# aredden/torch-bnb-fp4

Measured on AMD Instinct MI355X. Metric: FP4 dequant GB/s (% HBM peak) + fused-GEMV us/layer, 4096x4096 bf16, higher is better.
Workload: dtype bf16

## Files before the change

### torch-bnb-fp4_amd/csrc/gemv_common.h

```cpp
#pragma once

#include "fp4_common.h"

namespace fp4 {
namespace {

constexpr uint32_t kF16HiLo = 0x4A482C00u, kF16HiHi = 0x42404644u;
constexpr uint32_t kE4M3Lo = 0x54501800u, kE4M3Hi = 0x44404C48u;

__device__ __forceinline__ uint32_t perm(uint32_t hi, uint32_t lo, uint32_t sel) { return __builtin_amdgcn_perm(hi, lo, sel); }

template <int DT>
__device__ __forceinline__ void decode8(uint32_t q, uint32_t (&P)[4]) {
#if defined(FP4_EXP_BITOP3) || defined(FP4_EXP_RELAID)
    if constexpr (DT == FP4_DTYPE_BF16) {
        uint32_t m80;
        asm("v_mov_b32 %0, 0x80808080" : "=v"(m80));
        const uint32_t mhi = __builtin_amdgcn_bitop3_b32(q, m80, perm(kE4M3Hi, kE4M3Lo, (q >> 4) & 0x07070707u), 0xEA);
        const uint32_t mlo = __builtin_amdgcn_bitop3_b32(q << 4, m80, perm(kE4M3Hi, kE4M3Lo, q & 0x07070707u), 0xEA);
        P[0] = __builtin_bit_cast(uint32_t, __builtin_amdgcn_cvt_scalef32_pk_bf16_fp8(mhi, 1.0f, false));
        P[1] = __builtin_bit_cast(uint32_t, __builtin_amdgcn_cvt_scalef32_pk_bf16_fp8(mhi, 1.0f, true));
        P[2] = __builtin_bit_cast(uint32_t, __builtin_amdgcn_cvt_scalef32_pk_bf16_fp8(mlo, 1.0f, false));
        P[3] = __builtin_bit_cast(uint32_t, __builtin_amdgcn_cvt_scalef32_pk_bf16_fp8(mlo, 1.0f, true));
        return;
    }
#endif
    const uint32_t lo_sel = q & 0x07070707u;
    const uint32_t hi_sel = (q >> 4) & 0x07070707u;
    const uint32_t lo_sgn = (q & 0x08080808u) << 4;
    const uint32_t hi_sgn = q & 0x80808080u;
    if constexpr (DT == FP4_DTYPE_F16) {
        const uint32_t mhi = perm(kF16HiHi, kF16HiLo, hi_sel) | hi_sgn;
        const uint32_t mlo = perm(kF16HiHi, kF16HiLo, lo_sel) | lo_sgn;
        P[0] = perm(0u, mhi, 0x010C000Cu);
        P[1] = perm(0u, mhi, 0x030C020Cu);
        P[2] = perm(0u, mlo, 0x010C000Cu);
        P[3] = perm(0u, mlo, 0x030C020Cu);
    } else {
        const uint32_t mhi = perm(kE4M3Hi, kE4M3Lo, hi_sel) | hi_sgn;
        const uint32_t mlo = perm(kE4M3Hi, kE4M3Lo, lo_sel) | lo_sgn;
        P[0] = __builtin_bit_cast(uint32_t, __builtin_amdgcn_cvt_scalef32_pk_bf16_fp8(mhi, 1.0f, false));
        P[1] = __builtin_bit_cast(uint32_t, __builtin_amdgcn_cvt_scalef32_pk_bf16_fp8(mhi, 1.0f, true));
        P[2] = __builtin_bit_cast(uint32_t, __builtin_amdgcn_cvt_scalef32_pk_bf16_fp8(mlo, 1.0f, false));
        P[3] = __builtin_bit_cast(uint32_t, __builtin_amdgcn_cvt_scalef32_pk_bf16_fp8(mlo, 1.0f, true));
    }
}

template <int DT>
__device__ __forceinline__ float dot2(uint32_t a, uint32_t b, float c) {
    if constexpr (DT == FP4_DTYPE_F16)
        return __builtin_amdgcn_fdot2(__builtin_bit_cast(f16x2, a), __builtin_bit_cast(f16x2, b), c, false);
    else
        return __builtin_amdgcn_fdot2_f32_bf16(__builtin_bit_cast(bf16x2, a), __builtin_bit_cast(bf16x2, b), c, false);
}

template <int CTRL>
__device__ __forceinline__ float dpp_add(float v) {
    const int moved = __builtin_amdgcn_update_dpp(0, __builtin_bit_cast(int, v), CTRL, 0xF, 0xF, false);
    return v + __builtin_bit_cast(float, moved);
}
__device__ __forceinline__ float wave_sum(float v) {
    v = dpp_add<0x128>(v);
    v = dpp_add<0x124>(v);
    v = dpp_add<0x122>(v);
    v = dpp_add<0x121>(v);
    v += __builtin_bit_cast(float, __builtin_amdgcn_ds_swizzle(__builtin_bit_cast(int, v), 0x401F));
    const float a = __builtin_bit_cast(float, __builtin_amdgcn_readlane(__builtin_bit_cast(int, v), 0));
    const float b = __builtin_bit_cast(float, __builtin_amdgcn_readlane(__builtin_bit_cast(int, v), 32));
    return a + b;
}

constexpr int kModeOutF32 = 1;
constexpr int kModeSiluMulPairs = 2;

template <int DT>
__device__ __forceinline__ void store_row(uint16_t *out, const uint16_t *bias, const uint16_t *residual, int row, float sum,
                                          int mode = 0) {
    if (mode & kModeOutF32) {
        reinterpret_cast<float *>(out)[row] = sum;
        return;
    }
    uint16_t t = from_f32<DT>(sum);
    if (bias) t = from_f32<DT>(to_f32<DT>(t) + to_f32<DT>(bias[row]));
    if (residual) t = from_f32<DT>(to_f32<DT>(t) + to_f32<DT>(residual[row]));
    out[row] = t;
}

template <int DT>
__device__ __forceinline__ void store_silu_mul(uint16_t *out, const uint16_t *bias, const uint16_t *residual, int pair,
                                               float gate_sum, float up_sum) {
    uint16_t g = from_f32<DT>(gate_sum), u = from_f32<DT>(up_sum);
    if (bias) {
        g = from_f32<DT>(to_f32<DT>(g) + to_f32<DT>(bias[2 * pair]));
        u = from_f32<DT>(to_f32<DT>(u) + to_f32<DT>(bias[2 * pair + 1]));
    }
    const float gf = to_f32<DT>(g);
    const uint16_t s = from_f32<DT>(gf / (1.0f + expf(-gf)));
    uint16_t t = from_f32<DT>(to_f32<DT>(s) * to_f32<DT>(u));
    if (residual) t = from_f32<DT>(to_f32<DT>(t) + to_f32<DT>(residual[pair]));
    out[pair] = t;
}

template <int DT>
__device__ __forceinline__ void store_small(uint16_t *out, const uint16_t *bias, const uint16_t *residual, int64_t b, int row, int M,
                                            float sum) {
    if (bias) sum += to_f32<DT>(bias[row]);
    uint16_t t = from_f32<DT>(sum);
    if (residual) t = from_f32<DT>(to_f32<DT>(t) + to_f32<DT>(residual[b * M + row]));
    out[b * M + row] = t;
}

template <int DT>
__device__ __forceinline__ void store_small_silu_mul(uint16_t *out, const uint16_t *bias, const uint16_t *residual, int64_t b, int pair,
                                                     int M_half, float gate_sum, float up_sum) {
    if (bias) gate_sum += to_f32<DT>(bias[2 * pair]), up_sum += to_f32<DT>(bias[2 * pair + 1]);
    const float gf = to_f32<DT>(from_f32<DT>(gate_sum));
    const uint16_t s = from_f32<DT>(gf / (1.0f + expf(-gf)));
    uint16_t t = from_f32<DT>(to_f32<DT>(s) * to_f32<DT>(from_f32<DT>(up_sum)));
    if (residual) t = from_f32<DT>(to_f32<DT>(t) + to_f32<DT>(residual[b * M_half + pair]));
    out[b * M_half + pair] = t;
}

}
}
```

### torch-bnb-fp4_amd/csrc/gemv_fp4.hip

```cpp
#include <atomic>

#include "gemv_common.h"

#ifdef FP4_EXP_STAMPS
__device__ unsigned long long *fp4_exp_stamps = nullptr;
extern "C" int fp4_exp_set_stamps(void *buf) {
    return (int)hipMemcpyToSymbol(HIP_SYMBOL(fp4_exp_stamps), &buf, sizeof(buf));
}
#define FP4_STAMP(i)                                                                                        \
    do {                                                                                                    \
        __builtin_amdgcn_sched_barrier(0);                                                                  \
        const unsigned long long t_ = __builtin_amdgcn_s_memrealtime();                                     \
        if ((threadIdx.x & 63) == 0 && fp4_exp_stamps)                                                      \
            fp4_exp_stamps[(size_t(blockIdx.x) * WAVES + (threadIdx.x >> 6)) * 4 + (i)] = t_;               \
        __builtin_amdgcn_sched_barrier(0);                                                                  \
    } while (0)
#else
#define FP4_STAMP(i)
#endif

namespace fp4 {

namespace {

template <int ROWS, int UNROLL>
struct WTrip {
    u32x4 wq[UNROLL][ROWS];
    float am[UNROLL][ROWS];
};

template <int ROWS, int UNROLL>
__device__ __forceinline__ void issue_trip(WTrip<ROWS, UNROLL> &t, const u32x4 *__restrict__ Wv,
                                           const float *__restrict__ absmax, const int (&rows)[ROWS], int c0, int C,
                                           int bs_shift) {
#pragma unroll
    for (int u = 0; u < UNROLL; ++u) {
        const int c = c0 + 64 * u;
        const int cc = c < C ? c : C - 1;
#pragma unroll
        for (int r = 0; r < ROWS; ++r) {
            const int64_t chunk = int64_t(rows[r]) * C + cc;
            t.wq[u][r] = __builtin_nontemporal_load(Wv + chunk);
            const float a = absmax[(chunk << 5) >> bs_shift];
            t.am[u][r] = c < C ? a : 0.0f;
        }
    }
}

template <int DT, int ROWS, int UNROLL>
__device__ __forceinline__ void consume_trip(const WTrip<ROWS, UNROLL> &t, const u32x4 *s_x4, int c0, int C,
                                             float (&acc)[ROWS]) {
#pragma unroll
    for (int u = 0; u < UNROLL; ++u) {
        const int c = c0 + 64 * u;
        const int cc = c < C ? c : C - 1;
        u32x4 xd[4];
#pragma unroll
        for (int g = 0; g < 4; ++g) xd[g] = s_x4[g * C + cc];
#pragma unroll
        for (int r = 0; r < ROWS; ++r) {
            float s[4] = {0.0f, 0.0f, 0.0f, 0.0f};
#pragma unroll
            for (int g = 0; g < 4; ++g) {
                uint32_t P[4];
                decode8<DT>(t.wq[u][r][g], P);
                s[g] = dot2<DT>(P[0], xd[g].x, s[g]);
                s[g] = dot2<DT>(P[1], xd[g].y, s[g]);
                s[g] = dot2<DT>(P[2], xd[g].z, s[g]);
                s[g] = dot2<DT>(P[3], xd[g].w, s[g]);
            }
            acc[r] = __builtin_fmaf((s[0] + s[1]) + (s[2] + s[3]), t.am[u][r], acc[r]);
        }
    }
}

template <int DT, int ROWS, int WAVES, int UNROLL>
__global__ __launch_bounds__(WAVES * 64) void gemv16_kernel(const uint16_t *__restrict__ x,
                                                            const uint8_t *__restrict__ W,
                                                            const float *__restrict__ absmax,
                                                            const uint16_t *__restrict__ bias,
                                                            const uint16_t *residual, uint16_t *out, int M, int K,
                                                            int bs_shift, int mode) {
    extern __shared__ __attribute__((aligned(16))) uint32_t s_x[];
    u32x4 *s_x4 = reinterpret_cast<u32x4 *>(s_x);
    const int tid = threadIdx.x;
    const int lane = tid & 63;
    const int wave = tid >> 6;
    const int C = K >> 5;
    constexpr int kStride = 64 * UNROLL;
    const int trips = (C + kStride - 1) / kStride;

    const int row0 = (blockIdx.x * WAVES + wave) * ROWS;
    int rows[ROWS];
#pragma unroll
    for (int r = 0; r < ROWS; ++r) rows[r] = (row0 + r < M) ? row0 + r : M - 1;
    const u32x4 *Wv = reinterpret_cast<const u32x4 *>(W);

    constexpr int kXPre = 2;
    u32x4 xpre[kXPre];
#pragma unroll
    for (int i = 0; i < kXPre; ++i) {
        const int p = tid + i * WAVES * 64;
        xpre[i] = reinterpret_cast<const u32x4 *>(x)[p < 4 * C ? p : 4 * C - 1];
    }
    WTrip<ROWS, UNROLL> ta, tb;
    issue_trip<ROWS, UNROLL>(ta, Wv, absmax, rows, lane, C, bs_shift);

    auto stage = [&](int p, const u32x4 w) {
        u32x4 d;
        d.x = perm(w.y, w.x, 0x05040100u);
        d.y = perm(w.w, w.z, 0x05040100u);
        d.z = perm(w.y, w.x, 0x07060302u);
        d.w = perm(w.w, w.z, 0x07060302u);
        s_x4[(p & 3) * C + (p >> 2)] = d;
    };
#pragma unroll
    for (int i = 0; i < kXPre; ++i) {
        const int p = tid + i * WAVES * 64;
        if (p < 4 * C) stage(p, xpre[i]);
    }
    for (int p = tid + kXPre * WAVES * 64; p < 4 * C; p += WAVES * 64) stage(p, reinterpret_cast<const u32x4 *>(x)[p]);
    __syncthreads();

    float acc[ROWS];
#pragma unroll
    for (int r = 0; r < ROWS; ++r) acc[r] = 0.0f;

    for (int t = 0;;) {
        if (t + 1 < trips) issue_trip<ROWS, UNROLL>(tb, Wv, absmax, rows, lane + (t + 1) * kStride, C, bs_shift);
        consume_trip<DT, ROWS, UNROLL>(ta, s_x4, lane + t * kStride, C, acc);
        if (++t >= trips) break;
        if (t + 1 < trips) issue_trip<ROWS, UNROLL>(ta, Wv, absmax, rows, lane + (t + 1) * kStride, C, bs_shift);
        consume_trip<DT, ROWS, UNROLL>(tb, s_x4, lane + t * kStride, C, acc);
        if (++t >= trips) break;
    }

#pragma unroll
    for (int r = 0; r < ROWS; ++r) {
        const float total = wave_sum(acc[r]) * (1.0f / 12.0f);
        if (lane == 0 && row0 + r < M) store_row<DT>(out, bias, residual, row0 + r, total, mode);
    }
}

template <int DT, int KSPLIT, int G, int ITERS, int WAVES = 4>
__global__ __launch_bounds__(WAVES * 64, (G >= 4 ? 4 : 1)) void gemv16_regx_kernel(const uint16_t *__restrict__ x, const uint8_t *__restrict__ W,
                                                          const float *__restrict__ absmax,
                                                          const uint16_t *__restrict__ bias, const uint16_t *residual,
                                                          uint16_t *out, int M, int K, int bs_shift, int mode) {
    constexpr int RG = WAVES / KSPLIT;
    constexpr int kRowsPerBlock = 2 * RG * ITERS;
    __shared__ float s_part[kRowsPerBlock][KSPLIT];
    FP4_STAMP(0);
    const int tid = threadIdx.x;
    const int lane = tid & 63;
    const int wave = tid >> 6;
    const int kw = wave % KSPLIT, rw = wave / KSPLIT;
    const int half = lane >> 5, l32 = lane & 31;
    const int C = K >> 5;
    const int row_base = blockIdx.x * kRowsPerBlock;

    int cidx[G];
    bool live[G];
#pragma unroll
    for (int g = 0; g < G; ++g) {
        const int c = g * (32 * KSPLIT) + kw * 32 + l32;
        live[g] = c < C;
        cidx[g] = live[g] ? c : C - 1;
    }
    constexpr bool GMAJOR = G > 1;
    u32x4 xraw[G][4];
    u32x4 wq[ITERS][G];
    float am[ITERS][G];
    int rowi[ITERS], rclamp[ITERS];
#pragma unroll
    for (int it = 0; it < ITERS; ++it) {
        const int local = 2 * (it * RG + rw) + half;
        const int row = row_base + local;
        rowi[it] = local;
        rclamp[it] = row < M ? row : M - 1;
    }
    auto load_x = [&](int g) {
#pragma unroll
        for (int q = 0; q < 4; ++q) {
#ifdef FP4_ABL_NOX
            xraw[g][q] = u32x4{uint32_t(cidx[g]), 0x3c003c00u, uint32_t(q), 0x3c003c00u};
#else
            xraw[g][q] = reinterpret_cast<const u32x4 *>(x)[cidx[g] * 4 + q];
#endif
        }
    };
    const __amdgpu_buffer_rsrc_t rsrc_w = __builtin_amdgcn_make_buffer_rsrc(const_cast<uint8_t *>(W), 0, int((uint32_t(M) * uint32_t(C)) << 4), 0x00020000);
    const __amdgpu_buffer_rsrc_t rsrc_a =
        __builtin_amdgcn_make_buffer_rsrc(const_cast<float *>(absmax), 0, int(((uint32_t(M) * uint32_t(C)) >> (bs_shift - 5)) << 2), 0x00020000);
    auto load_w = [&](int it, int g) {
        const uint32_t chunk = uint32_t(rclamp[it]) * uint32_t(C) + uint32_t(cidx[g]);
        wq[it][g] = __builtin_bit_cast(u32x4, __builtin_amdgcn_raw_buffer_load_b128(rsrc_w, int(chunk << 4), 0, 2));
#ifdef FP4_ABL_NOABSMAX
        const float a = 0.5f;
#else
        const float a = __builtin_bit_cast(float, __builtin_amdgcn_raw_buffer_load_b32(rsrc_a, int((chunk >> (bs_shift - 5)) << 2), 0, 0));
#endif
        am[it][g] = live[g] ? a : 0.0f;
    };
    if constexpr (GMAJOR) {
#pragma unroll
        for (int g = 0; g < G; ++g) {
            load_x(g);
#pragma unroll
            for (int it = 0; it < ITERS; ++it) load_w(it, g);
        }
    } else {
#pragma unroll
        for (int g = 0; g < G; ++g) load_x(g);
#pragma unroll
        for (int it = 0; it < ITERS; ++it) {
#pragma unroll
            for (int g = 0; g < G; ++g) load_w(it, g);
        }
    }
    FP4_STAMP(1);
    u32x4 xd[G][4];
    auto permute_x = [&](int g) {
#pragma unroll
        for (int q = 0; q < 4; ++q) {
            const u32x4 w = xraw[g][q];
#ifdef FP4_EXP_RELAID
            xd[g][q] = u32x4{w.x, w.z, w.y, w.w};
#else
            xd[g][q].x = perm(w.y, w.x, 0x05040100u);
            xd[g][q].y = perm(w.w, w.z, 0x05040100u);
            xd[g][q].z = perm(w.y, w.x, 0x07060302u);
            xd[g][q].w = perm(w.w, w.z, 0x07060302u);
#endif
        }
    };
    if constexpr (!GMAJOR) {
#pragma unroll
        for (int g = 0; g < G; ++g) permute_x(g);
    }
    float pacc[ITERS];
#pragma unroll
    for (int it = 0; it < ITERS; ++it) pacc[it] = 0.0f;
    auto consume = [&](int it, int g) {
        float s[2] = {0.0f, 0.0f};
#ifdef FP4_ABL_NOCOMPUTE
#pragma unroll
        for (int q = 0; q < 4; ++q) s[q & 1] = __builtin_bit_cast(float, (wq[it][g][q] ^ xd[g][q].x) & 0x3fffffffu);
#else
#pragma unroll
        for (int q = 0; q < 4; ++q) {
            uint32_t P[4];
            decode8<DT>(wq[it][g][q], P);
            s[q & 1] = dot2<DT>(P[0], xd[g][q].x, s[q & 1]);
            s[q & 1] = dot2<DT>(P[1], xd[g][q].y, s[q & 1]);
            s[q & 1] = dot2<DT>(P[2], xd[g][q].z, s[q & 1]);
            s[q & 1] = dot2<DT>(P[3], xd[g][q].w, s[q & 1]);
        }
#endif
        pacc[it] = __builtin_fmaf(s[0] + s[1], am[it][g], pacc[it]);
    };
    if constexpr (GMAJOR) {
#pragma unroll
        for (int g = 0; g < G; ++g) {
            permute_x(g);
#pragma unroll
            for (int it = 0; it < ITERS; ++it) consume(it, g);
            __builtin_amdgcn_sched_barrier(0);
        }
    } else {
#pragma unroll
        for (int it = 0; it < ITERS; ++it) {
#pragma unroll
            for (int g = 0; g < G; ++g) consume(it, g);
        }
    }
    FP4_STAMP(2);
#pragma unroll
    for (int it = 0; it < ITERS; ++it) {
        float p = pacc[it];
        p = dpp_add<0x128>(p);
        p = dpp_add<0x124>(p);
        p = dpp_add<0x122>(p);
        p = dpp_add<0x121>(p);
        p += __builtin_bit_cast(float, __builtin_amdgcn_ds_swizzle(__builtin_bit_cast(int, p), 0x401F));
        if constexpr (KSPLIT == 1) {
            const int row = row_base + rowi[it];
            if (mode & kModeSiluMulPairs) {
                const float up = __builtin_bit_cast(float, __builtin_amdgcn_readlane(__builtin_bit_cast(int, p), 32));
                if (lane == 0 && row < M) store_silu_mul<DT>(out, bias, residual, row >> 1, p * (1.0f / 12.0f), up * (1.0f / 12.0f));
            } else if (l32 == 0 && row < M) {
                store_row<DT>(out, bias, residual, row, p * (1.0f / 12.0f), mode);
            }
        } else {
            if (l32 == 0) s_part[rowi[it]][kw] = p;
        }
    }
    if constexpr (KSPLIT > 1) {
        __syncthreads();
        if (mode & kModeSiluMulPairs) {
            if (tid < kRowsPerBlock / 2) {
                float g = 0.0f, u = 0.0f;
#pragma unroll
                for (int k = 0; k < KSPLIT; ++k) g += s_part[2 * tid][k], u += s_part[2 * tid + 1][k];
                const int row = row_base + 2 * tid;
                if (row < M) store_silu_mul<DT>(out, bias, residual, row >> 1, g * (1.0f / 12.0f), u * (1.0f / 12.0f));
            }
        } else if (tid < kRowsPerBlock) {
            float t = 0.0f;
#pragma unroll
            for (int k = 0; k < KSPLIT; ++k) t += s_part[tid][k];
            const int row = row_base + tid;
            if (row < M) store_row<DT>(out, bias, residual, row, t * (1.0f / 12.0f), mode);
        }
    }
    FP4_STAMP(3);
}

template <int ROWS, int WAVES>
__global__ __launch_bounds__(WAVES * 64) void gemv32_kernel(const float *__restrict__ x, const uint8_t *__restrict__ W,
                                                            const float *__restrict__ absmax,
                                                            const float *__restrict__ bias, const float *residual, float *out,
                                                            int M, int K, int bs_shift) {
    extern __shared__ __attribute__((aligned(16))) uint32_t s_raw[];
    f32x4 *s_x4 = reinterpret_cast<f32x4 *>(s_raw);
    __shared__ float s_lut[16];
    const int tid = threadIdx.x;
    const int lane = tid & 63;
    const int wave = tid >> 6;
    const int C = K >> 5;

    if (tid < 16) s_lut[tid] = lut_entry(FP4_TABLE_CODEBOOK, tid);
    for (int p = tid; p < 8 * C; p += WAVES * 64) s_x4[(p & 7) * C + (p >> 3)] = reinterpret_cast<const f32x4 *>(x)[p];
    __syncthreads();

    const int row0 = (blockIdx.x * WAVES + wave) * ROWS;
    if (row0 >= M) return;
    int rows[ROWS];
#pragma unroll
    for (int r = 0; r < ROWS; ++r) rows[r] = (row0 + r < M) ? row0 + r : M - 1;

    const u32x4 *Wv = reinterpret_cast<const u32x4 *>(W);
    float acc[ROWS];
#pragma unroll
    for (int r = 0; r < ROWS; ++r) acc[r] = 0.0f;

    for (int c = lane; c < C; c += 64) {
        u32x4 wq[ROWS];
        float am[ROWS];
#pragma unroll
        for (int r = 0; r < ROWS; ++r) {
            const int64_t chunk = int64_t(rows[r]) * C + c;
            wq[r] = __builtin_nontemporal_load(Wv + chunk);
            am[r] = absmax[(chunk << 5) >> bs_shift];
        }
        float s[ROWS];
#pragma unroll
        for (int r = 0; r < ROWS; ++r) s[r] = 0.0f;
#pragma unroll
        for (int g = 0; g < 8; ++g) {
            const f32x4 xv = s_x4[g * C + c];
#pragma unroll
            for (int r = 0; r < ROWS; ++r) {
                const uint32_t h = (wq[r][g >> 1] >> (16 * (g & 1))) & 0xFFFFu;
                s[r] = __builtin_fmaf(s_lut[(h >> 4) & 15u], xv.x, s[r]);
                s[r] = __builtin_fmaf(s_lut[h & 15u], xv.y, s[r]);
                s[r] = __builtin_fmaf(s_lut[(h >> 12) & 15u], xv.z, s[r]);
                s[r] = __builtin_fmaf(s_lut[(h >> 8) & 15u], xv.w, s[r]);
            }
        }
#pragma unroll
        for (int r = 0; r < ROWS; ++r) acc[r] = __builtin_fmaf(s[r], am[r], acc[r]);
    }
#pragma unroll
    for (int r = 0; r < ROWS; ++r) {
        const float total = wave_sum(acc[r]);
        if (lane == 0 && row0 + r < M) {
            const float t = bias ? total + bias[row0 + r] : total;
            out[row0 + r] = residual ? t + residual[row0 + r] : t;
        }
    }
}

template <int KSPLIT, int G, int ITERS>
__global__ __launch_bounds__(256) void gemv32_regx_kernel(const float *__restrict__ x, const uint8_t *__restrict__ W,
                                                          const float *__restrict__ absmax, const float *__restrict__ bias,
                                                          const float *residual, float *out, int M, int K, int bs_shift) {
    constexpr int RG = 4 / KSPLIT;
    constexpr int kRowsPerBlock = 2 * RG * ITERS;
    __shared__ float s_lut[16];
    __shared__ float s_part[kRowsPerBlock][KSPLIT];
    const int tid = threadIdx.x;
    const int lane = tid & 63;
    const int wave = tid >> 6;
    const int kw = wave % KSPLIT, rw = wave / KSPLIT;
    const int half = lane >> 5, l32 = lane & 31;
    const int C = K >> 5;
    const int row_base = blockIdx.x * kRowsPerBlock;
    const u32x4 *Wv = reinterpret_cast<const u32x4 *>(W);
    if (tid < 16) s_lut[tid] = lut_entry(FP4_TABLE_CODEBOOK, tid);

    int cidx[G];
    bool live[G];
#pragma unroll
    for (int g = 0; g < G; ++g) {
        const int c = g * (32 * KSPLIT) + kw * 32 + l32;
        live[g] = c < C;
        cidx[g] = live[g] ? c : C - 1;
    }
    f32x4 xv[G][8];
#pragma unroll
    for (int g = 0; g < G; ++g) {
#pragma unroll
        for (int q = 0; q < 8; ++q) xv[g][q] = reinterpret_cast<const f32x4 *>(x)[cidx[g] * 8 + q];
    }
    u32x4 wq[ITERS][G];
    float am[ITERS][G];
    int rowi[ITERS];
#pragma unroll
    for (int it = 0; it < ITERS; ++it) {
        const int local = 2 * (it * RG + rw) + half;
        const int row = row_base + local;
        rowi[it] = local;
        const int rclamp = row < M ? row : M - 1;
#pragma unroll
        for (int g = 0; g < G; ++g) {
            const int64_t chunk = int64_t(rclamp) * C + cidx[g];
            wq[it][g] = __builtin_nontemporal_load(Wv + chunk);
            const float a = absmax[(chunk << 5) >> bs_shift];
            am[it][g] = live[g] ? a : 0.0f;
        }
    }
    __syncthreads();
#pragma unroll
    for (int it = 0; it < ITERS; ++it) {
        float p = 0.0f;
#pragma unroll
        for (int g = 0; g < G; ++g) {
            float s0 = 0.0f, s1 = 0.0f;
#pragma unroll
            for (int q = 0; q < 8; ++q) {
                const uint32_t h = (wq[it][g][q >> 1] >> (16 * (q & 1))) & 0xFFFFu;
                s0 = __builtin_fmaf(s_lut[(h >> 4) & 15u], xv[g][q].x, s0);
                s1 = __builtin_fmaf(s_lut[h & 15u], xv[g][q].y, s1);
                s0 = __builtin_fmaf(s_lut[(h >> 12) & 15u], xv[g][q].z, s0);
                s1 = __builtin_fmaf(s_lut[(h >> 8) & 15u], xv[g][q].w, s1);
            }
            p = __builtin_fmaf(s0 + s1, am[it][g], p);
        }
        p = dpp_add<0x128>(p);
        p = dpp_add<0x124>(p);
        p = dpp_add<0x122>(p);
        p = dpp_add<0x121>(p);
        p += __builtin_bit_cast(float, __builtin_amdgcn_ds_swizzle(__builtin_bit_cast(int, p), 0x401F));
        if constexpr (KSPLIT == 1) {
            const int row = row_base + rowi[it];
            if (l32 == 0 && row < M) {
                const float t = bias ? p + bias[row] : p;
                out[row] = residual ? t + residual[row] : t;
            }
        } else {
            if (l32 == 0) s_part[rowi[it]][kw] = p;
        }
    }
    if constexpr (KSPLIT > 1) {
        __syncthreads();
        if (tid < kRowsPerBlock) {
            float t = 0.0f;
#pragma unroll
            for (int k = 0; k < KSPLIT; ++k) t += s_part[tid][k];
            const int row = row_base + tid;
            if (row < M) {
                t = bias ? t + bias[row] : t;
                out[row] = residual ? t + residual[row] : t;
            }
        }
    }
}

template <int KSPLIT, int G, int ITERS>
int launch32_regx(const void *x, const uint8_t *W, const float *absmax, const void *bias, const void *residual, void *out, int M,
                  int K, int bs_shift, hipStream_t stream) {
    constexpr int rows_per_block = 2 * (4 / KSPLIT) * ITERS;
    const unsigned blocks = (unsigned)((M + rows_per_block - 1) / rows_per_block);
    hipLaunchKernelGGL((gemv32_regx_kernel<KSPLIT, G, ITERS>), dim3(blocks), dim3(256), 0, stream,
                       reinterpret_cast<const float *>(x), W, absmax, reinterpret_cast<const float *>(bias),
                       reinterpret_cast<const float *>(residual), reinterpret_cast<float *>(out), M, K, bs_shift);
    return FP4_OK;
}

int dispatch32_regx(int iters, const void *x, const uint8_t *W, const float *absmax, const void *bias, const void *residual, void *out,
                    int M, int K, int bs_shift, hipStream_t stream) {
    const int C = K >> 5;
    const int ks = C <= 32 ? 1 : (C <= 64 ? 2 : 4);
    if (iters <= 0) {
        iters = 1;
        while (iters < 4 && M / (2 * (4 / ks) * iters * 2) >= 256) iters *= 2;
    }
#define FP4_R32(KS, GG)                                                                                                   \
    switch (iters) {                                                                                                      \
        case 1: return launch32_regx<KS, GG, 1>(x, W, absmax, bias, residual, out, M, K, bs_shift, stream);        \
        case 2: return launch32_regx<KS, GG, 2>(x, W, absmax, bias, residual, out, M, K, bs_shift, stream);        \
        default: return launch32_regx<KS, GG, 4>(x, W, absmax, bias, residual, out, M, K, bs_shift, stream);       \
    }
    if (C <= 32) { FP4_R32(1, 1) }
    if (C <= 64) { FP4_R32(2, 1) }
    if (C <= 128) { FP4_R32(4, 1) }
    if (C <= 256) { FP4_R32(4, 2) }
#undef FP4_R32
    return -1;
}

template <int DT>
__global__ __launch_bounds__(256) void gemv_generic_kernel(const void *__restrict__ xv, const uint8_t *__restrict__ W,
                                                           const float *__restrict__ absmax, const void *__restrict__ biasv,
                                                           const void *residualv, void *outv, int M, int64_t K, int blocksize,
                                                           CodeTable tbl, int mode) {
    const int lane = threadIdx.x & 63;
    const int row = blockIdx.x * 4 + (threadIdx.x >> 6);
    if (row >= M) return;
    const int64_t e_row = int64_t(row) * K;
    float acc = 0.0f;
    for (int64_t b = lane; b < K / 2; b += 64) {
        const int64_t e = e_row + 2 * b;
        const uint32_t q = W[e >> 1];
        const float am = absmax[e / blocksize];
        float x0, x1;
        if constexpr (DT == FP4_DTYPE_F32) {
            x0 = reinterpret_cast<const float *>(xv)[2 * b];
            x1 = reinterpret_cast<const float *>(xv)[2 * b + 1];
        } else {
            x0 = to_f32<DT>(reinterpret_cast<const uint16_t *>(xv)[2 * b]);
            x1 = to_f32<DT>(reinterpret_cast<const uint16_t *>(xv)[2 * b + 1]);
        }
        acc = __builtin_fmaf(__builtin_bit_cast(float, tbl.bits[q >> 4]) * am, x0, acc);
        acc = __builtin_fmaf(__builtin_bit_cast(float, tbl.bits[q & 15u]) * am, x1, acc);
    }
    const float total = wave_sum(acc);
    if (lane == 0) {
        if constexpr (DT == FP4_DTYPE_F32) {
            const float *bias = reinterpret_cast<const float *>(biasv), *residual = reinterpret_cast<const float *>(residualv);
            const float t = bias ? total + bias[row] : total;
            reinterpret_cast<float *>(outv)[row] = residual ? t + residual[row] : t;
        } else {
            store_row<DT>(reinterpret_cast<uint16_t *>(outv), reinterpret_cast<const uint16_t *>(biasv),
                          reinterpret_cast<const uint16_t *>(residualv), row, total, mode);
        }
    }
}

std::atomic<int> g_gemv_variant{-1};

constexpr int kMaxLdsBytes = 160 * 1024 - 256;

template <typename Kern>
int ensure_lds(Kern kern, size_t lds_bytes) {
    if (lds_bytes <= 64 * 1024) return FP4_OK;
    if (hipFuncSetAttribute(reinterpret_cast<const void *>(kern), hipFuncAttributeMaxDynamicSharedMemorySize,
                            (int)lds_bytes) != hipSuccess) {
        (void)hipGetLastError();
        set_error("fp4_hip_gemv: cannot reserve %zu bytes of LDS", lds_bytes);
        return FP4_ERR_UNSUPPORTED;
    }
    return FP4_OK;
}

struct GemvArgs {
    const void *x;
    const uint8_t *W;
    const float *absmax;
    const void *bias, *residual;
    void *out;
    int M, K, bs_shift, mode;
    hipStream_t stream;
};

template <int DT, int ROWS, int WAVES, int UNROLL>
int launch16(const GemvArgs &a) {
    if (a.mode & kModeSiluMulPairs) return -2;
    auto kern = gemv16_kernel<DT, ROWS, WAVES, UNROLL>;
    const int M = a.M, K = a.K;
    const size_t lds = size_t(K) * 2;
    if (int rc = ensure_lds(kern, lds)) return rc;
    const int rows_per_block = ROWS * WAVES;
    const unsigned blocks = (unsigned)((M + rows_per_block - 1) / rows_per_block);
    hipLaunchKernelGGL(kern, dim3(blocks), dim3(WAVES * 64), lds, a.stream, reinterpret_cast<const uint16_t *>(a.x), a.W, a.absmax,
                       reinterpret_cast<const uint16_t *>(a.bias), reinterpret_cast<const uint16_t *>(a.residual),
                       reinterpret_cast<uint16_t *>(a.out), M, K, a.bs_shift, a.mode);
    return FP4_OK;
}

template <int DT>
int dispatch16(int variant, const GemvArgs &a) {
    switch (variant) {
#define FP4_V(R, Wv, U)                  \
    case (R | (Wv << 8) | (U << 16)):    \
        return launch16<DT, R, Wv, U>(a);
        FP4_V(1, 4, 2) FP4_V(1, 8, 2)
#undef FP4_V
        default:
            set_error("fp4_hip_gemv: unknown kernel variant 0x%x", variant);
            return FP4_ERR_INVALID_ARGUMENT;
    }
}

constexpr int kRegxFlag = 1 << 24;

template <int DT, int KSPLIT, int G, int ITERS, int WAVES = 4>
int launch_regx(const GemvArgs &a) {
    constexpr int rows_per_block = 2 * (WAVES / KSPLIT) * ITERS;
    const unsigned blocks = (unsigned)((a.M + rows_per_block - 1) / rows_per_block);
    hipLaunchKernelGGL((gemv16_regx_kernel<DT, KSPLIT, G, ITERS, WAVES>), dim3(blocks), dim3(WAVES * 64), 0, a.stream,
                       reinterpret_cast<const uint16_t *>(a.x), a.W, a.absmax, reinterpret_cast<const uint16_t *>(a.bias),
                       reinterpret_cast<const uint16_t *>(a.residual), reinterpret_cast<uint16_t *>(a.out), a.M, a.K, a.bs_shift,
                       a.mode);
    return FP4_OK;
}

template <int DT>
int dispatch_regx(int iters, int ks_override, const GemvArgs &a) {
    const int C = a.K >> 5;
    if (int64_t(a.M) * a.K >= (int64_t(1) << 32)) return -1;
    if (ks_override == 7 && C % 224 == 0 && (C / 224 == 1 || C / 224 == 2 || C / 224 == 4)) {
        const int g7 = C / 224;
        if (g7 == 1) return launch_regx<DT, 7, 1, 2, 7>(a);
        if (g7 == 2) return launch_regx<DT, 7, 2, 4, 7>(a);
        return launch_regx<DT, 7, 4, 2, 7>(a);
    }
    if ((ks_override == 5 && C % 160 == 0 && C / 160 <= 2) || (ks_override == 6 && C == 192)) {
        const int gg = C / (32 * ks_override);
        if (iters > 4) iters = 4;
#define FP4_RXN(KS, GG)                                                                                               \
    switch (iters) {                                                                                                  \
        case 1: return launch_regx<DT, KS, GG, 1, KS>(a);      \
        case 2: return launch_regx<DT, KS, GG, 2, KS>(a);      \
        default: return launch_regx<DT, KS, GG, 4, KS>(a);     \
    }
        if (ks_override == 5 && gg == 1) { FP4_RXN(5, 1) }
        if (ks_override == 5 && gg == 2) { FP4_RXN(5, 2) }
        if (ks_override == 6 && gg == 1) { FP4_RXN(6, 1) }
#undef FP4_RXN
    }
    if (ks_override == 8 && C == 256) {
        if (iters >= 4) return launch_regx<DT, 8, 1, 4, 8>(a);
        return launch_regx<DT, 8, 1, 2, 8>(a);
    }
    const int ks = C <= 32 ? 1 : (C <= 64 ? 2 : 4);
    const int need = (C + 32 * ks - 1) / (32 * ks);
    const int g = need <= 1 ? 1 : (need <= 2 ? 2 : ((need == 3 && ks == 4) ? 3 : (need <= 4 ? 4 : 0)));
    if (g == 0) return -1;
    if (iters > 4) iters = 4;
    if (g >= 3 && iters > 2) iters = 2;
    if (iters == 3) iters = 2;
    if (iters < 1) iters = 1;
#define FP4_RX(KS, GG, IT) return launch_regx<DT, KS, GG, IT>(a)
#define FP4_RX_IT(KS, GG)                                    \
    if (ks == KS && g == GG) {                               \
        switch (iters) {                                     \
            case 1: FP4_RX(KS, GG, 1);                       \
            case 2: FP4_RX(KS, GG, 2);                       \
            case 4:                                          \
                if constexpr ((GG) <= 2) { FP4_RX(KS, GG, 4); } \
                break;                                       \
            default: break;                                  \
        }                                                    \
    }
    FP4_RX_IT(1, 1) FP4_RX_IT(2, 1) FP4_RX_IT(4, 1) FP4_RX_IT(4, 2) FP4_RX_IT(4, 3) FP4_RX_IT(4, 4)
#undef FP4_RX_IT
#undef FP4_RX
    set_error("fp4_hip_gemv: unknown regx geometry (iters %d, ksplit %d, g %d)", iters, ks, g);
    return FP4_ERR_INVALID_ARGUMENT;
}

int default_variant16(int M, int K) {
    const int C = K >> 5;
    if (C == 160 || C == 320 || C == 192) {
        int it = 1;
        while (it * 2 <= 4 && M / (2 * it * 2) >= 1024) it *= 2;
        return kRegxFlag | ((C == 192 ? 6 : 5) << 8) | it;
    }
    if (C == 256 && M >= 4096) {
        int it = 1;
        while (it * 2 <= 4 && M / (2 * it * 2) >= 1024) it *= 2;
        return kRegxFlag | (8 << 8) | it;
    }
    if (C == 224) return kRegxFlag | (7 << 8) | 2;
    if (C == 448 && M <= 4096) return kRegxFlag | (7 << 8) | 4;
    if (C == 896) return kRegxFlag | (7 << 8) | 2;
    const int ksplit = C <= 32 ? 1 : (C <= 64 ? 2 : 4);
    const int rows_per_iter = 2 * (4 / ksplit);
    const int max_iters = C <= 128 ? 4 : (C <= 256 ? 4 : 2);
    int iters = 1;
    if (max_iters >= 2 && M / (rows_per_iter * 2) >= 1024) iters = 2;
    if (max_iters >= 4 && M / (rows_per_iter * 4) >= 2048) iters = 4;
    return kRegxFlag | iters;
}

template <int DT>
int run_generic(const void *x, const uint8_t *W, const float *absmax, const void *bias, const void *residual, void *out, int64_t M,
                int64_t K, int blocksize, int mode, hipStream_t stream, int table = FP4_TABLE_CODEBOOK) {
    const CodeTable tbl = make_table(table);
    hipLaunchKernelGGL((gemv_generic_kernel<DT>), dim3((unsigned)((M + 3) / 4)), dim3(256), 0, stream, x, W, absmax, bias,
                       residual, out, (int)M, K, blocksize, tbl, mode);
    return FP4_OK;
}

}

void set_gemv_variant(int v) { g_gemv_variant.store(v, std::memory_order_relaxed); }

int gemv_generic_table(const void *x, const uint8_t *W, const float *absmax, const void *bias, void *out, int64_t M, int64_t K,
                       int blocksize, int dtype, int table, hipStream_t stream) {
    switch (dtype) {
        case FP4_DTYPE_F16: return run_generic<FP4_DTYPE_F16>(x, W, absmax, bias, nullptr, out, M, K, blocksize, 0, stream, table);
        case FP4_DTYPE_BF16: return run_generic<FP4_DTYPE_BF16>(x, W, absmax, bias, nullptr, out, M, K, blocksize, 0, stream, table);
        default: return run_generic<FP4_DTYPE_F32>(x, W, absmax, bias, nullptr, out, M, K, blocksize, 0, stream, table);
    }
}

}

namespace fp4 {
namespace {
int gemv_entry(const void *x, const uint8_t *packed, const float *absmax, const void *bias, const void *residual, void *out,
               int64_t M, int64_t K, int blocksize, int dtype, int mode, void *stream) {
    if (M < 0 || K < 0 || (K & 1) || blocksize < 2 || (blocksize & 1)) {
        set_error("fp4_hip_gemv: M=%lld K=%lld blocksize=%d (need M,K >= 0, even K, even blocksize >= 2)", (long long)M,
                  (long long)K, blocksize);
        return FP4_ERR_INVALID_ARGUMENT;
    }
    if (dtype != FP4_DTYPE_F16 && dtype != FP4_DTYPE_BF16 && dtype != FP4_DTYPE_F32) {
        set_error("fp4_hip_gemv: unsupported dtype %d", dtype);
        return FP4_ERR_UNSUPPORTED;
    }
    if ((mode & kModeSiluMulPairs) && (M & 1)) {
        set_error("fp4_hip_gemv_fused: the gate|up epilogue needs an even row count, got M=%lld", (long long)M);
        return FP4_ERR_INVALID_ARGUMENT;
    }
    if (M == 0) return FP4_OK;
    if (!out || (K > 0 && (!x || !packed || !absmax))) {
        set_error("fp4_hip_gemv: null pointer");
        return FP4_ERR_INVALID_ARGUMENT;
    }
    if (M > (int64_t(1) << 30) || K > (int64_t(1) << 30)) {
        set_error("fp4_hip_gemv: M=%lld K=%lld too large", (long long)M, (long long)K);
        return FP4_ERR_UNSUPPORTED;
    }
    hipStream_t s = static_cast<hipStream_t>(stream);
    const int bs_shift = ilog2_exact(blocksize);
    const uintptr_t align = reinterpret_cast<uintptr_t>(packed) | reinterpret_cast<uintptr_t>(x);
    const size_t esz = dtype == FP4_DTYPE_F32 ? 4 : 2;
    const bool fast = K > 0 && (K % 32) == 0 && bs_shift >= 5 && (K % blocksize) == 0 && (align & 15u) == 0 &&
                      size_t(K) * esz <= size_t(kMaxLdsBytes);
    int rc = FP4_OK;
    const int gv = g_gemv_variant.load(std::memory_order_relaxed);
    if (fast && dtype != FP4_DTYPE_F32) {
        const GemvArgs a{x, packed, absmax, bias, residual, out, (int)M, (int)K, bs_shift, mode, s};
        int variant = gv >= 0 ? gv : default_variant16((int)M, (int)K);
        rc = -1;
        if (variant & kRegxFlag) {
            const int iters = variant & 0xFF, ks_override = (variant >> 8) & 0xF;
            rc = dtype == FP4_DTYPE_F16 ? dispatch_regx<FP4_DTYPE_F16>(iters, ks_override, a)
                                        : dispatch_regx<FP4_DTYPE_BF16>(iters, ks_override, a);
            if (rc == -1) variant = 1 | (8 << 8) | (2 << 16);
        }
        if (rc == -1) rc = dtype == FP4_DTYPE_F16 ? dispatch16<FP4_DTYPE_F16>(variant, a) : dispatch16<FP4_DTYPE_BF16>(variant, a);
    } else if (mode & kModeSiluMulPairs) {
        rc = -2;
    } else if (fast && gv != 0 &&
               dispatch32_regx(gv < 0 ? 0 : (gv & 0xFF), x, packed, absmax, bias, residual, out, (int)M, (int)K, bs_shift, s) == FP4_OK) {
        rc = FP4_OK;
    } else if (fast) {
        auto kern = gemv32_kernel<1, 4>;
        const size_t lds = size_t(K) * 4;
        rc = ensure_lds(kern, lds);
        if (rc == FP4_OK)
            hipLaunchKernelGGL(kern, dim3((unsigned)((M + 3) / 4)), dim3(256), lds, s, reinterpret_cast<const float *>(x),
                               packed, absmax, reinterpret_cast<const float *>(bias), reinterpret_cast<const float *>(residual),
                               reinterpret_cast<float *>(out), (int)M, (int)K, bs_shift);
    } else {
        switch (dtype) {
            case FP4_DTYPE_F16:
                rc = run_generic<FP4_DTYPE_F16>(x, packed, absmax, bias, residual, out, M, K, blocksize, mode, s);
                break;
            case FP4_DTYPE_BF16:
                rc = run_generic<FP4_DTYPE_BF16>(x, packed, absmax, bias, residual, out, M, K, blocksize, mode, s);
                break;
            default:
                rc = run_generic<FP4_DTYPE_F32>(x, packed, absmax, bias, residual, out, M, K, blocksize, mode, s);
                break;
        }
    }
    if (rc == -2) {
        set_error("fp4_hip_gemv_fused: the gate|up epilogue is not available for M=%lld K=%lld blocksize=%d dtype=%d "
                  "(needs a 16-bit dtype, K %% 32 == 0, K <= 16384 or 28672, a power-of-two blocksize >= 32 that divides K); run the plain GEMV and "
                  "apply the activation separately", (long long)M, (long long)K, blocksize, dtype);
        return FP4_ERR_UNSUPPORTED;
    }
    if (rc != FP4_OK) return rc;
    return check_launch("fp4_hip_gemv");
}
}
}

extern "C" int fp4_hip_gemv(const void *x, const uint8_t *packed, const float *absmax, const void *bias, void *out,
                            int64_t M, int64_t K, int blocksize, int dtype, void *stream) {
    return fp4::gemv_entry(x, packed, absmax, bias, nullptr, out, M, K, blocksize, dtype, 0, stream);
}

extern "C" int fp4_hip_gemv_fused(const void *x, const uint8_t *packed, const float *absmax, const void *bias, const void *residual,
                                  void *out, int64_t M, int64_t K, int blocksize, int dtype, int epilogue, void *stream) {
    if (epilogue != FP4_EPILOGUE_NONE && epilogue != FP4_EPILOGUE_SILU_MUL_PAIRS) {
        fp4::set_error("fp4_hip_gemv_fused: unknown epilogue %d", epilogue);
        return FP4_ERR_INVALID_ARGUMENT;
    }
    return fp4::gemv_entry(x, packed, absmax, bias, residual, out, M, K, blocksize, dtype,
                           epilogue == FP4_EPILOGUE_SILU_MUL_PAIRS ? fp4::kModeSiluMulPairs : 0, stream);
}

extern "C" int fp4_hip_gemv_partial(const void *x, const uint8_t *packed, const float *absmax, float *out_f32, int64_t M,
                                    int64_t K, int blocksize, int x_dtype, void *stream) {
    return fp4::gemv_entry(x, packed, absmax, nullptr, nullptr, out_f32, M, K, blocksize, x_dtype, fp4::kModeOutF32, stream);
}
```

Baseline: 5943.

## Halve per-lane x loads via permlane32 swap, hoist epilogue loads, vectorize stores

Each lane now loads only half of the x vector chunk and rebuilds the full chunk with permlane32_swap, which cuts redundant x traffic. In the G-major path the absmax loads are issued ahead of the weight loads. Bias and residual values are prefetched with buffer loads before the main loop so they are not fetched in the epilogue. The cross-lane reduction is restructured: DPP steps are interleaved across rows, and a row_pair DPP add replaces ds_swizzle, so outputs now come from lanes 16 and 48. KSPLIT outputs are packed across lanes into 32/64-bit stores. Together these add register pressure, more cross-lane operations and extra code complexity.

```diff
diff --git a/torch-bnb-fp4_amd/csrc/gemv_common.h b/torch-bnb-fp4_amd/csrc/gemv_common.h
--- a/torch-bnb-fp4_amd/csrc/gemv_common.h
+++ b/torch-bnb-fp4_amd/csrc/gemv_common.h
@@ -70,6 +70,11 @@
     return a + b;
 }
 
+__device__ __forceinline__ float row_pair_sum_hi(float v) {
+    const int moved = __builtin_amdgcn_update_dpp(0, __builtin_bit_cast(int, v), 0x142, 0xA, 0xF, false);
+    return v + __builtin_bit_cast(float, moved);
+}
+
 constexpr int kModeOutF32 = 1;
 constexpr int kModeSiluMulPairs = 2;
 
@@ -101,6 +106,55 @@
     out[pair] = t;
 }
 
+__device__ __forceinline__ uint16_t buffer_load_u16(__amdgpu_buffer_rsrc_t rsrc, int byte_offset) {
+    return __builtin_bit_cast(uint16_t, __builtin_amdgcn_raw_buffer_load_b16(rsrc, byte_offset, 0, 0));
+}
+
+template <int DT>
+__device__ __forceinline__ uint16_t finish_row(float sum, bool has_bias, uint16_t b, bool has_residual, uint16_t r) {
+    uint16_t t = from_f32<DT>(sum);
+    if (has_bias) t = from_f32<DT>(to_f32<DT>(t) + to_f32<DT>(b));
+    if (has_residual) t = from_f32<DT>(to_f32<DT>(t) + to_f32<DT>(r));
+    return t;
+}
+
+template <int DT>
+__device__ __forceinline__ uint16_t finish_silu_mul(float gate_sum, float up_sum, bool has_bias, uint16_t bg, uint16_t bu,
+                                                    bool has_residual, uint16_t r) {
+    uint16_t g = from_f32<DT>(gate_sum), u = from_f32<DT>(up_sum);
+    if (has_bias) {
+        g = from_f32<DT>(to_f32<DT>(g) + to_f32<DT>(bg));
+        u = from_f32<DT>(to_f32<DT>(u) + to_f32<DT>(bu));
+    }
+    const float gf = to_f32<DT>(g);
+    const uint16_t s = from_f32<DT>(gf / (1.0f + expf(-gf)));
+    uint16_t t = from_f32<DT>(to_f32<DT>(s) * to_f32<DT>(u));
+    if (has_residual) t = from_f32<DT>(to_f32<DT>(t) + to_f32<DT>(r));
+    return t;
+}
+
+template <int N>
+__device__ __forceinline__ void store_lanes(uint16_t *out, int idx0, int lane, uint16_t t, bool whole, bool mine) {
+    constexpr int W = N % 4 == 0 ? 4 : (N % 2 == 0 ? 2 : 1);
+    if constexpr (W > 1) {
+        if (whole) {
+            const uint32_t w0 = uint32_t(t) | uint32_t(__builtin_amdgcn_update_dpp(0, int(t), 0xF5, 0xF, 0xF, true)) << 16;
+            if constexpr (W == 2) {
+                if ((lane & 1) == 0) *reinterpret_cast<uint32_t *>(out + idx0 + lane) = w0;
+            } else {
+                const uint32_t w1 = uint32_t(__builtin_amdgcn_update_dpp(0, int(w0), 0xAA, 0xF, 0xF, true));
+#ifdef FP4_EXP_WT
+                if ((lane & 3) == 0) __hip_atomic_store(reinterpret_cast<uint64_t *>(out + idx0 + lane), uint64_t(w0) | uint64_t(w1) << 32, __ATOMIC_RELAXED, __HIP_MEMORY_SCOPE_AGENT);
+#else
+                if ((lane & 3) == 0) *reinterpret_cast<u32x2 *>(out + idx0 + lane) = u32x2{w0, w1};
+#endif
+            }
+            return;
+        }
+    }
+    if (mine) out[idx0 + lane] = t;
+}
+
 template <int DT>
 __device__ __forceinline__ void store_small(uint16_t *out, const uint16_t *bias, const uint16_t *residual, int64_t b, int row, int M,
                                             float sum) {
diff --git a/torch-bnb-fp4_amd/csrc/gemv_fp4.hip b/torch-bnb-fp4_amd/csrc/gemv_fp4.hip
--- a/torch-bnb-fp4_amd/csrc/gemv_fp4.hip
+++ b/torch-bnb-fp4_amd/csrc/gemv_fp4.hip
@@ -7,16 +7,22 @@
 extern "C" int fp4_exp_set_stamps(void *buf) {
     return (int)hipMemcpyToSymbol(HIP_SYMBOL(fp4_exp_stamps), &buf, sizeof(buf));
 }
-#define FP4_STAMP(i)                                                                                        \
+#define FP4_STAMP_SLOTS 6
+#define FP4_STAMP_PUT(i, value)                                                                             \
     do {                                                                                                    \
         __builtin_amdgcn_sched_barrier(0);                                                                  \
-        const unsigned long long t_ = __builtin_amdgcn_s_memrealtime();                                     \
+        const unsigned long long t_ = (value);                                                              \
         if ((threadIdx.x & 63) == 0 && fp4_exp_stamps)                                                      \
-            fp4_exp_stamps[(size_t(blockIdx.x) * WAVES + (threadIdx.x >> 6)) * 4 + (i)] = t_;               \
+            fp4_exp_stamps[(size_t(blockIdx.x) * WAVES + (threadIdx.x >> 6)) * FP4_STAMP_SLOTS + (i)] = t_; \
         __builtin_amdgcn_sched_barrier(0);                                                                  \
     } while (0)
+#define FP4_STAMP(i) FP4_STAMP_PUT(i, __builtin_amdgcn_s_memrealtime())
+#define FP4_STAMP_WHERE()                                                                                   \
+    FP4_STAMP_PUT(5, (unsigned long long)(uint32_t)__builtin_amdgcn_s_getreg(4 | (31 << 11)) |              \
+                         (unsigned long long)(uint32_t)__builtin_amdgcn_s_getreg(20 | (31 << 11)) << 32)
 #else
 #define FP4_STAMP(i)
+#define FP4_STAMP_WHERE()
 #endif
 
 namespace fp4 {
@@ -151,6 +157,7 @@
     constexpr int kRowsPerBlock = 2 * RG * ITERS;
     __shared__ float s_part[kRowsPerBlock][KSPLIT];
     FP4_STAMP(0);
+    FP4_STAMP_WHERE();
     const int tid = threadIdx.x;
     const int lane = tid & 63;
     const int wave = tid >> 6;
@@ -168,7 +175,11 @@
         cidx[g] = live[g] ? c : C - 1;
     }
     constexpr bool GMAJOR = G > 1;
+#ifdef FP4_EXP_X4
     u32x4 xraw[G][4];
+#else
+    u32x4 xraw[G][2];
+#endif
     u32x4 wq[ITERS][G];
     float am[ITERS][G];
     int rowi[ITERS], rclamp[ITERS];
@@ -181,27 +192,57 @@
     }
     auto load_x = [&](int g) {
 #pragma unroll
-        for (int q = 0; q < 4; ++q) {
+#ifdef FP4_EXP_X4
+        for (int q = 0; q < 4; ++q) xraw[g][q] = reinterpret_cast<const u32x4 *>(x)[cidx[g] * 4 + q];
+#else
+        for (int q = 0; q < 2; ++q) {
 #ifdef FP4_ABL_NOX
             xraw[g][q] = u32x4{uint32_t(cidx[g]), 0x3c003c00u, uint32_t(q), 0x3c003c00u};
 #else
-            xraw[g][q] = reinterpret_cast<const u32x4 *>(x)[cidx[g] * 4 + q];
-#endif
-        }
+            xraw[g][q] = reinterpret_cast<const u32x4 *>(x)[cidx[g] * 4 + 2 * half + q];
+#endif
+        }
+#endif
     };
     const __amdgpu_buffer_rsrc_t rsrc_w = __builtin_amdgcn_make_buffer_rsrc(const_cast<uint8_t *>(W), 0, int((uint32_t(M) * uint32_t(C)) << 4), 0x00020000);
     const __amdgpu_buffer_rsrc_t rsrc_a =
         __builtin_amdgcn_make_buffer_rsrc(const_cast<float *>(absmax), 0, int(((uint32_t(M) * uint32_t(C)) >> (bs_shift - 5)) << 2), 0x00020000);
+    auto load_a = [&](int it, int g) {
+#ifdef FP4_ABL_NOABSMAX
+        am[it][g] = live[g] ? 0.5f : 0.0f;
+#else
+        const uint32_t chunk = uint32_t(rclamp[it]) * uint32_t(C) + uint32_t(cidx[g]);
+        am[it][g] = __builtin_bit_cast(float, __builtin_amdgcn_raw_buffer_load_b32(rsrc_a, live[g] ? int((chunk >> (bs_shift - 5)) << 2) : -1, 0, 0));
+#endif
+    };
     auto load_w = [&](int it, int g) {
         const uint32_t chunk = uint32_t(rclamp[it]) * uint32_t(C) + uint32_t(cidx[g]);
         wq[it][g] = __builtin_bit_cast(u32x4, __builtin_amdgcn_raw_buffer_load_b128(rsrc_w, int(chunk << 4), 0, 2));
-#ifdef FP4_ABL_NOABSMAX
-        const float a = 0.5f;
-#else
-        const float a = __builtin_bit_cast(float, __builtin_amdgcn_raw_buffer_load_b32(rsrc_a, int((chunk >> (bs_shift - 5)) << 2), 0, 0));
-#endif
-        am[it][g] = live[g] ? a : 0.0f;
+        if constexpr (!GMAJOR) load_a(it, g);
     };
+    const bool gated = mode & kModeSiluMulPairs;
+    uint16_t bias0 = 0, bias1 = 0, res = 0;
+    if constexpr (KSPLIT > 1) {
+        if (__builtin_amdgcn_readfirstlane(wave) == 0 && !(mode & kModeOutF32) && (bias || residual)) {
+            const int e = (gated ? row_base >> 1 : row_base) + tid;
+            const bool fin = tid < (gated ? kRowsPerBlock / 2 : kRowsPerBlock);
+            const __amdgpu_buffer_rsrc_t rsrc_b = __builtin_amdgcn_make_buffer_rsrc(const_cast<uint16_t *>(bias), 0, bias ? 2 * M : 0, 0x00020000);
+            const __amdgpu_buffer_rsrc_t rsrc_b1 = __builtin_amdgcn_make_buffer_rsrc(const_cast<uint16_t *>(bias), 0, bias && gated ? 2 * M : 0, 0x00020000);
+            const __amdgpu_buffer_rsrc_t rsrc_r =
+                __builtin_amdgcn_make_buffer_rsrc(const_cast<uint16_t *>(residual), 0, residual ? (gated ? M : 2 * M) : 0, 0x00020000);
+            bias0 = buffer_load_u16(rsrc_b, fin ? e << (gated ? 2 : 1) : -1);
+            bias1 = buffer_load_u16(rsrc_b1, fin ? 4 * e + 2 : -1);
+            res = buffer_load_u16(rsrc_r, fin ? 2 * e : -1);
+        }
+    }
+    if constexpr (GMAJOR) {
+#pragma unroll
+        for (int it = 0; it < ITERS; ++it) {
+#pragma unroll
+            for (int g = 0; g < G; ++g) load_a(it, g);
+        }
+        __builtin_amdgcn_sched_barrier(0);
+    }
     if constexpr (GMAJOR) {
 #pragma unroll
         for (int g = 0; g < G; ++g) {
@@ -210,20 +251,47 @@
             for (int it = 0; it < ITERS; ++it) load_w(it, g);
         }
     } else {
+#ifdef FP4_EXP_WFIRST
+#pragma unroll
+        for (int it = 0; it < ITERS; ++it) {
+#pragma unroll
+            for (int g = 0; g < G; ++g) load_w(it, g);
+        }
+        __builtin_amdgcn_sched_barrier(0);
 #pragma unroll
         for (int g = 0; g < G; ++g) load_x(g);
+#else
+#pragma unroll
+        for (int g = 0; g < G; ++g) load_x(g);
 #pragma unroll
         for (int it = 0; it < ITERS; ++it) {
 #pragma unroll
             for (int g = 0; g < G; ++g) load_w(it, g);
         }
-    }
+#endif
+    }
+    __builtin_amdgcn_sched_barrier(0);
     FP4_STAMP(1);
     u32x4 xd[G][4];
     auto permute_x = [&](int g) {
+        u32x4 xfull[4];
+#ifdef FP4_EXP_X4
+#pragma unroll
+        for (int q = 0; q < 4; ++q) xfull[q] = xraw[g][q];
+#else
+#pragma unroll
+        for (int q = 0; q < 2; ++q) {
+#pragma unroll
+            for (int d = 0; d < 4; ++d) {
+                const auto sw = __builtin_amdgcn_permlane32_swap(xraw[g][q][d], xraw[g][q][d], false, false);
+                xfull[q][d] = sw[0];
+                xfull[q + 2][d] = sw[1];
+            }
+        }
+#endif
 #pragma unroll
         for (int q = 0; q < 4; ++q) {
-            const u32x4 w = xraw[g][q];
+            const u32x4 w = xfull[q];
 #ifdef FP4_EXP_RELAID
             xd[g][q] = u32x4{w.x, w.z, w.y, w.w};
 #else
@@ -275,45 +343,72 @@
         }
     }
     FP4_STAMP(2);
+    __builtin_amdgcn_sched_barrier(0);
+#pragma unroll
+    for (int it = 0; it < ITERS; ++it) pacc[it] = dpp_add<0x128>(pacc[it]);
+#pragma unroll
+    for (int it = 0; it < ITERS; ++it) pacc[it] = dpp_add<0x124>(pacc[it]);
+#pragma unroll
+    for (int it = 0; it < ITERS; ++it) pacc[it] = dpp_add<0x122>(pacc[it]);
+#pragma unroll
+    for (int it = 0; it < ITERS; ++it) pacc[it] = dpp_add<0x121>(pacc[it]);
 #pragma unroll
     for (int it = 0; it < ITERS; ++it) {
-        float p = pacc[it];
-        p = dpp_add<0x128>(p);
-        p = dpp_add<0x124>(p);
-        p = dpp_add<0x122>(p);
-        p = dpp_add<0x121>(p);
-        p += __builtin_bit_cast(float, __builtin_amdgcn_ds_swizzle(__builtin_bit_cast(int, p), 0x401F));
-        if constexpr (KSPLIT == 1) {
+#ifdef FP4_EXP_SWZ
+        pacc[it] += __builtin_bit_cast(float, __builtin_amdgcn_ds_swizzle(__builtin_bit_cast(int, pacc[it]), 0x401F));
+#else
+        pacc[it] = row_pair_sum_hi(pacc[it]);
+#endif
+    }
+    if constexpr (KSPLIT == 1) {
+#pragma unroll
+        for (int it = 0; it < ITERS; ++it) {
+            const float p = pacc[it];
             const int row = row_base + rowi[it];
-            if (mode & kModeSiluMulPairs) {
-                const float up = __builtin_bit_cast(float, __builtin_amdgcn_readlane(__builtin_bit_cast(int, p), 32));
-                if (lane == 0 && row < M) store_silu_mul<DT>(out, bias, residual, row >> 1, p * (1.0f / 12.0f), up * (1.0f / 12.0f));
-            } else if (l32 == 0 && row < M) {
+            if (gated) {
+                const float up = __builtin_bit_cast(float, __builtin_amdgcn_readlane(__builtin_bit_cast(int, p), 48));
+                if (lane == 16 && row < M) store_silu_mul<DT>(out, bias, residual, row >> 1, p * (1.0f / 12.0f), up * (1.0f / 12.0f));
+            } else if (l32 == 16 && row < M) {
                 store_row<DT>(out, bias, residual, row, p * (1.0f / 12.0f), mode);
             }
-        } else {
-            if (l32 == 0) s_part[rowi[it]][kw] = p;
-        }
-    }
-    if constexpr (KSPLIT > 1) {
+        }
+    } else {
+        if (l32 == 16) {
+#pragma unroll
+            for (int it = 0; it < ITERS; ++it) s_part[rowi[it]][kw] = pacc[it];
+        }
         __syncthreads();
-        if (mode & kModeSiluMulPairs) {
+        FP4_STAMP(3);
+        uint32_t b0 = bias0, b1 = bias1, rs = res;
+        asm volatile("" : "+v"(b0), "+v"(b1), "+v"(rs));
+        bias0 = uint16_t(b0), bias1 = uint16_t(b1), res = uint16_t(rs);
+#ifdef FP4_EXP_NOGATHER
+        const bool whole = false;
+#else
+        const bool whole = row_base + kRowsPerBlock <= M && (reinterpret_cast<uintptr_t>(out) & 7u) == 0;
+#endif
+        if (gated) {
             if (tid < kRowsPerBlock / 2) {
                 float g = 0.0f, u = 0.0f;
 #pragma unroll
                 for (int k = 0; k < KSPLIT; ++k) g += s_part[2 * tid][k], u += s_part[2 * tid + 1][k];
-                const int row = row_base + 2 * tid;
-                if (row < M) store_silu_mul<DT>(out, bias, residual, row >> 1, g * (1.0f / 12.0f), u * (1.0f / 12.0f));
+                const uint16_t t = finish_silu_mul<DT>(g * (1.0f / 12.0f), u * (1.0f / 12.0f), bias != nullptr, bias0, bias1, residual != nullptr, res);
+                store_lanes<kRowsPerBlock / 2>(out, row_base >> 1, tid, t, whole, row_base + 2 * tid < M);
             }
         } else if (tid < kRowsPerBlock) {
             float t = 0.0f;
 #pragma unroll
             for (int k = 0; k < KSPLIT; ++k) t += s_part[tid][k];
+            t *= 1.0f / 12.0f;
             const int row = row_base + tid;
-            if (row < M) store_row<DT>(out, bias, residual, row, t * (1.0f / 12.0f), mode);
-        }
-    }
-    FP4_STAMP(3);
+            if (mode & kModeOutF32) {
+                if (row < M) reinterpret_cast<float *>(out)[row] = t;
+            } else {
+                store_lanes<kRowsPerBlock>(out, row_base, tid, finish_row<DT>(t, bias != nullptr, bias0, residual != nullptr, res), whole, row < M);
+            }
+        }
+    }
+    FP4_STAMP(4);
 }
 
 template <int ROWS, int WAVES>
```

New measurement: 5944 (median of 6 runs). About the same (+0.0%).
